# arkworks-rs/poly-commit

Measured on NVIDIA H100. Metric: MarlinKZG10/BLS12-381 commit+open polys/s at deg 2^20, higher is better.
Workload: dtype u32-limb Montgomery (Fq 381-bit x12, Fr 255-bit x8)

## Files before the change

poly-commit_b200/csrc/msm.cuh:

```cuda
#pragma once
#include "ec.cuh"
#include "rt.cuh"

namespace pcgpu {

struct alignas(16) u32x4 { uint32_t x, y, z, w; };

struct MsmGeom {
  uint32_t n;
  uint32_t c;
  uint32_t W;
  uint32_t S;
  uint32_t G;
  uint32_t NB;
  uint32_t TB;
  uint32_t L;
  uint32_t seg_len;
  uint32_t nseg;
  uint32_t scalar_bits;
  uint32_t scalars_mont;
  uint64_t table_stride;
  uint64_t base_off;
  uint32_t affine_rounds;
  uint32_t h_split;
  uint32_t pt_words;
  uint32_t y_words;
  uint32_t pair_tdiv;
};

enum : uint32_t { ENTRY_SIGN = 0x80000000u, ENTRY_GROUP_SHIFT = 26, ENTRY_IDX_MASK = (1u << 26) - 1 };

template <class C>
PCGPU_DEV void load_scalar_plain(const uint32_t *scalars, size_t i, bool mont, uint32_t *k) {
  using R = typename C::Fr;
  const u32x4 *p = reinterpret_cast<const u32x4 *>(scalars) + 2 * i;
  u32x4 lo = p[0], hi = p[1];
  Fp<R> v;
  v.l[0] = lo.x; v.l[1] = lo.y; v.l[2] = lo.z; v.l[3] = lo.w;
  v.l[4] = hi.x; v.l[5] = hi.y; v.l[6] = hi.z; v.l[7] = hi.w;
  if (mont) v = fp_from_mont<R>(v);
#pragma unroll
  for (int j = 0; j < 8; j++) k[j] = v.l[j];
}

template <class C>
PCGPU_DEV bool load_scalar(const uint32_t *scalars, size_t i, bool mont, uint32_t *k, bool *flip) {
  using R = typename C::Fr;
  static_assert(R::N == 8, "256-bit scalar fields only");
  const u32x4 *p = reinterpret_cast<const u32x4 *>(scalars) + 2 * i;
  u32x4 lo = p[0], hi = p[1];
  Fp<R> v;
  v.l[0] = lo.x; v.l[1] = lo.y; v.l[2] = lo.z; v.l[3] = lo.w;
  v.l[4] = hi.x; v.l[5] = hi.y; v.l[6] = hi.z; v.l[7] = hi.w;
  if (mont) v = fp_from_mont<R>(v);
  bool lt_r = false, gt_half = false, decided_r = false, decided_h = false;
#pragma unroll
  for (int j = 7; j >= 0; j--) {
    const uint32_t m = R::mod(j), h = (R::mod(j) >> 1) | (j + 1 < 8 ? R::mod(j + 1 < 8 ? j + 1 : 7) << 31 : 0u);
    if (!decided_r && v.l[j] != m) { lt_r = v.l[j] < m; decided_r = true; }
    if (!decided_h && v.l[j] != h) { gt_half = v.l[j] > h; decided_h = true; }
  }
  *flip = gt_half;
  if (gt_half) {
    Fp<R> m;
#pragma unroll
    for (int j = 0; j < 8; j++) m.l[j] = R::mod(j);
    uint32_t borrow = 0;
#pragma unroll
    for (int j = 0; j < 8; j++) {
      const uint64_t dd = (uint64_t)m.l[j] - v.l[j] - borrow;
      v.l[j] = (uint32_t)dd; borrow = (uint32_t)(dd >> 63);
    }
  }
#pragma unroll
  for (int j = 0; j < 8; j++) k[j] = v.l[j];
  return lt_r;
}

PCGPU_DEV uint32_t scalar_bits_at(const uint32_t *k, uint32_t pos, uint32_t c) {
  uint32_t q = pos >> 5, sh = pos & 31;
  uint64_t lo = q < 8 ? k[q] : 0u;
  uint64_t hi = q + 1 < 8 ? k[q + 1] : 0u;
  uint64_t v = (lo | (hi << 32)) >> sh;
  return (uint32_t)v & ((1u << c) - 1);
}

template <class Fn>
PCGPU_DEV void for_each_digit(const uint32_t *k, const MsmGeom &g, Fn f) {
  uint32_t carry = 0;
  const uint32_t half = 1u << (g.c - 1);
  for (uint32_t w = 0; w < g.W; w++) {
    uint32_t d = scalar_bits_at(k, w * g.c, g.c) + carry;
    bool neg = d > half;
    carry = neg ? 1u : 0u;
    uint32_t mag = neg ? (1u << g.c) - d : d;
    if (mag) f(w, mag, neg);
  }
}

PCGPU_DEV bool scalar_in_range(const uint32_t *k, uint32_t bits) {
  if (bits >= 256) return true;
  uint32_t q = bits >> 5, sh = bits & 31;
  uint32_t o = k[q] >> sh;
  for (uint32_t j = q + 1; j < 8; j++) o |= k[j];
  return o == 0;
}

template <class C>
struct MsmCountBody {
  const uint32_t *scalars; MsmGeom g; uint32_t *counts; uint32_t *err;
  PCGPU_KERNEL_DEV void operator()(size_t i) const {
    uint32_t k[8];
    bool flip;
    if (!load_scalar<C>(scalars, i, g.scalars_mont != 0, k, &flip)) { rt::atomic_or(err, 1u); return; }
    uint32_t *cnt = counts; const MsmGeom gg = g;
    for_each_digit(k, gg, [&](uint32_t w, uint32_t mag, bool) {
      uint32_t s = w % gg.S;
      rt::atomic_add(cnt + (size_t)s * gg.NB + (mag - 1), 1u);
    });
  }
};

template <class C>
struct MsmScatterBody {
  const uint32_t *scalars; MsmGeom g; uint32_t *cursor; uint32_t *entries;
  PCGPU_KERNEL_DEV void operator()(size_t i) const {
    uint32_t k[8];
    bool flip;
    if (!load_scalar<C>(scalars, i, g.scalars_mont != 0, k, &flip)) return;
    uint32_t *cur = cursor; uint32_t *ent = entries; const MsmGeom gg = g;
    for_each_digit(k, gg, [&](uint32_t w, uint32_t mag, bool neg) {
      uint32_t s = w % gg.S, grp = w / gg.S;
      uint32_t pos = rt::atomic_add(cur + (size_t)s * gg.NB + (mag - 1), 1u);
      ent[pos] = ((neg != flip) ? ENTRY_SIGN : 0u) | (grp << ENTRY_GROUP_SHIFT) | (uint32_t)i;
    });
  }
};

enum { SCAN_CHUNK = 256 };
struct ScanChunkSumBody {
  const uint32_t *in; size_t n; uint32_t *partial;
  PCGPU_KERNEL_DEV void operator()(size_t t) const {
    size_t lo = t * SCAN_CHUNK, hi = lo + SCAN_CHUNK < n ? lo + SCAN_CHUNK : n;
    uint32_t s = 0;
    for (size_t i = lo; i < hi; i++) s += in[i];
    partial[t] = s;
  }
};
struct ScanPartialsBody {
  uint32_t *partial; size_t m;
  PCGPU_KERNEL_DEV void operator()(size_t) const {
    uint32_t run = 0;
    for (size_t i = 0; i < m; i++) { uint32_t v = partial[i]; partial[i] = run; run += v; }
    partial[m] = run;
  }
};
struct ScanApplyBody {
  const uint32_t *in; size_t n; const uint32_t *partial; uint32_t *out; size_t m;
  PCGPU_KERNEL_DEV void operator()(size_t t) const {
    size_t lo = t * SCAN_CHUNK, hi = lo + SCAN_CHUNK < n ? lo + SCAN_CHUNK : n;
    uint32_t run = partial[t];
    for (size_t i = lo; i < hi; i++) { uint32_t v = in[i]; out[i] = run; run += v; }
    if (t + 1 == m) out[n] = partial[m];
  }
};

enum { SCAN_BLOCK = 1024, SCAN_PER = 8, SCAN_BLOCK_MAX = 1 << 17 };
struct ScanBlockBody {
  const uint32_t *in; size_t n; uint32_t *out;
  PCGPU_KERNEL_DEV void operator()(size_t, uint32_t *smem) const {
    uint32_t *a = smem, *b = smem + SCAN_BLOCK, *carry = smem + 2 * SCAN_BLOCK;
    PCGPU_BLOCK_FOR(t, 1) { carry[0] = 0; }
    PCGPU_BLOCK_SYNC();
    const size_t tile = (size_t)SCAN_BLOCK * SCAN_PER;
    for (size_t base = 0; base < n; base += tile) {
      PCGPU_BLOCK_FOR(t, SCAN_BLOCK) {
        const size_t lo = base + (size_t)t * SCAN_PER;
        uint32_t sum = 0;
        for (uint32_t k = 0; k < SCAN_PER; k++) if (lo + k < n) sum += in[lo + k];
        a[t] = sum;
      }
      PCGPU_BLOCK_SYNC();
      uint32_t *x = a, *y = b;
      for (uint32_t d = 1; d < SCAN_BLOCK; d <<= 1) {
        PCGPU_BLOCK_FOR(t, SCAN_BLOCK) { y[t] = x[t] + (t >= d ? x[t - d] : 0u); }
        PCGPU_BLOCK_SYNC();
        uint32_t *tmp = x; x = y; y = tmp;
      }
      PCGPU_BLOCK_FOR(t, SCAN_BLOCK) {
        const size_t lo = base + (size_t)t * SCAN_PER;
        uint32_t run = carry[0] + (t ? x[t - 1] : 0u);
        for (uint32_t k = 0; k < SCAN_PER; k++) if (lo + k < n) { uint32_t v = in[lo + k]; out[lo + k] = run; run += v; }
      }
      PCGPU_BLOCK_SYNC();
      PCGPU_BLOCK_FOR(t, 1) { carry[0] += x[SCAN_BLOCK - 1]; }
      PCGPU_BLOCK_SYNC();
    }
    PCGPU_BLOCK_FOR(t, 1) { out[n] = carry[0]; }
  }
};

inline size_t scan_scratch_words(size_t n) { return (n + SCAN_CHUNK - 1) / SCAN_CHUNK + 2; }
inline int exclusive_scan_u32(const uint32_t *in, size_t n, uint32_t *out, uint32_t *scratch, rt::stream_t st) {
  size_t m = (n + SCAN_CHUNK - 1) / SCAN_CHUNK;
  if (m == 0) { return rt::dev_memset(out, 0, sizeof(uint32_t), st); }
  if (n <= SCAN_BLOCK_MAX) return rt::launch_blocks<SCAN_BLOCK>(ScanBlockBody{in, n, out}, 1, (2 * SCAN_BLOCK + 4) * sizeof(uint32_t), st);
  int rc;
  if ((rc = rt::launch<128>(ScanChunkSumBody{in, n, scratch}, m, st))) return rc;
  if ((rc = rt::launch<32>(ScanPartialsBody{scratch, m}, 1, st))) return rc;
  return rt::launch<128>(ScanApplyBody{in, n, scratch, out, m}, m, st);
}

struct TaskCountBody {
  const uint32_t *offsets; uint32_t L; uint32_t *ntasks; uint32_t heavy_min; uint32_t *heavy_count; uint32_t *heavy_list;
  PCGPU_KERNEL_DEV void operator()(size_t b) const {
    uint32_t cnt = offsets[b + 1] - offsets[b];
    uint32_t nt = (cnt + L - 1) / L;
    ntasks[b] = nt;
    if (nt > heavy_min) heavy_list[rt::atomic_add(heavy_count, 1u)] = (uint32_t)b;
  }
};
struct TaskFillBody {
  const uint32_t *task_off; uint32_t *task_bucket;
  PCGPU_KERNEL_DEV void operator()(size_t b) const {
    uint32_t lo = task_off[b], hi = task_off[b + 1];
    for (uint32_t t = lo; t < hi; t++) task_bucket[t] = (uint32_t)b;
  }
};

template <class C>
PCGPU_DEV Affine<C> load_affine(const Affine<C> *p) {
  constexpr int N = coord_words<typename C::F>();
  const u32x4 *q = reinterpret_cast<const u32x4 *>(p);
  Affine<C> a;
  uint32_t tmp[2 * N];
#pragma unroll
  for (int j = 0; j < 2 * N / 4; j++) { u32x4 v = q[j]; tmp[4 * j] = v.x; tmp[4 * j + 1] = v.y; tmp[4 * j + 2] = v.z; tmp[4 * j + 3] = v.w; }
#pragma unroll
  for (int j = 0; j < N; j++) {
    if constexpr (C::EXT == 1) { a.x.l[j] = tmp[j]; a.y.l[j] = tmp[N + j]; }
    else { coord_word(a.x, j) = tmp[j]; coord_word(a.y, j) = tmp[N + j]; }
  }
  return a;
}

template <class C>
PCGPU_DEV const uint32_t *table_record(const uint32_t *tables, size_t idx, const MsmGeom &g) { return tables + idx * g.pt_words; }
template <class C>
PCGPU_DEV Affine<C> load_table_point(const uint32_t *tables, size_t idx, const MsmGeom &g) {
  constexpr int N = coord_words<typename C::F>();
  const uint32_t *rec = tables + idx * g.pt_words;
  const u32x4 *qx = reinterpret_cast<const u32x4 *>(rec), *qy = reinterpret_cast<const u32x4 *>(rec + g.y_words);
  Affine<C> a;
#pragma unroll
  for (int j = 0; j < N / 4; j++) {
    u32x4 v = qx[j]; coord_word(a.x, 4 * j) = v.x; coord_word(a.x, 4 * j + 1) = v.y; coord_word(a.x, 4 * j + 2) = v.z; coord_word(a.x, 4 * j + 3) = v.w;
    u32x4 w = qy[j]; coord_word(a.y, 4 * j) = w.x; coord_word(a.y, 4 * j + 1) = w.y; coord_word(a.y, 4 * j + 2) = w.z; coord_word(a.y, 4 * j + 3) = w.w;
  }
  return a;
}
template <class C>
PCGPU_DEV void store_table_point(uint32_t *tables, size_t idx, uint32_t pt_words, uint32_t y_words, const Affine<C> &a) {
  constexpr int N = coord_words<typename C::F>();
  uint32_t *rec = tables + idx * pt_words;
  u32x4 *qx = reinterpret_cast<u32x4 *>(rec), *qy = reinterpret_cast<u32x4 *>(rec + y_words);
#pragma unroll
  for (int j = 0; j < N / 4; j++) {
    u32x4 v; v.x = coord_word(a.x, 4 * j); v.y = coord_word(a.x, 4 * j + 1); v.z = coord_word(a.x, 4 * j + 2); v.w = coord_word(a.x, 4 * j + 3); qx[j] = v;
    u32x4 w; w.x = coord_word(a.y, 4 * j); w.y = coord_word(a.y, 4 * j + 1); w.z = coord_word(a.y, 4 * j + 2); w.w = coord_word(a.y, 4 * j + 3); qy[j] = w;
  }
}
template <class C> constexpr uint32_t aligned_pt_words() { return C::Fq::N == 12 ? 32u : 2u * C::Fq::N; }
template <class C> constexpr uint32_t aligned_y_words() { return C::Fq::N == 12 ? 16u : (uint32_t)C::Fq::N; }

template <class C>
PCGPU_DEV void store_xyzz(XYZZ<C> *dst, const XYZZ<C> &p) {
  constexpr int N = coord_words<typename C::F>();
  u32x4 *q = reinterpret_cast<u32x4 *>(dst);
  const uint32_t *src = reinterpret_cast<const uint32_t *>(&p);
#pragma unroll
  for (int j = 0; j < 4 * N / 4; j++) { u32x4 v; v.x = src[4 * j]; v.y = src[4 * j + 1]; v.z = src[4 * j + 2]; v.w = src[4 * j + 3]; q[j] = v; }
}

template <class C>
PCGPU_DEV XYZZ<C> load_xyzz(const XYZZ<C> *src) {
  constexpr int N = coord_words<typename C::F>();
  const u32x4 *q = reinterpret_cast<const u32x4 *>(src);
  XYZZ<C> p;
  uint32_t *dst = reinterpret_cast<uint32_t *>(&p);
#pragma unroll
  for (int j = 0; j < 4 * N / 4; j++) { u32x4 v = q[j]; dst[4 * j] = v.x; dst[4 * j + 1] = v.y; dst[4 * j + 2] = v.z; dst[4 * j + 3] = v.w; }
  return p;
}

template <class C>
struct MsmAccumulateBody {
  const uint32_t *tables; MsmGeom g;
  const uint32_t *offsets;
  const uint32_t *task_off;
  const uint32_t *task_bucket;
  const uint32_t *entries;
  XYZZ<C> *partial;
  uint32_t *queue;
  const Affine<C> *pts;
  PCGPU_KERNEL_DEV void operator()(size_t) const {
    const uint32_t total = task_off[g.TB];
    for (;;) {
      uint32_t t = rt::next_task(queue);
      if (t - (t & 31u) >= total) break;
      if (t >= total) continue;
      uint32_t b = task_bucket[t];
      uint32_t t0 = task_off[b], T = task_off[b + 1] - t0, j = t - t0;
      uint32_t base = offsets[b], cnt = offsets[b + 1] - base;
      uint32_t lo = base + (uint32_t)(((uint64_t)cnt * j) / T);
      uint32_t hi = base + (uint32_t)(((uint64_t)cnt * (j + 1)) / T);
      XYZZ<C> acc = XYZZ<C>::inf();
      if (pts) {
        for (uint32_t e = lo; e < hi; e++) { Affine<C> a = load_affine<C>(pts + e); xyzz_madd<C>(acc, a, false); }
      } else {
        for (uint32_t e = lo; e < hi; e++) {
          uint32_t v = entries[e];
          uint32_t grp = (v & ~ENTRY_SIGN) >> ENTRY_GROUP_SHIFT;
          size_t idx = (size_t)grp * g.table_stride + g.base_off + (v & ENTRY_IDX_MASK);
          Affine<C> a = load_table_point<C>(tables, idx, g);
          xyzz_madd<C>(acc, a, (v & ENTRY_SIGN) != 0);
        }
      }
      store_xyzz<C>(partial + t, acc);
    }
  }
};

enum { HEAVY_BUCKET_TASKS = 8, HEAVY_BLOCK = 128, HEAVY_GRID = 64, REDUCE_BLOCK = 128 };

template <class C>
#ifdef __CUDACC__
__device__ __noinline__
#else
inline
#endif
void xyzz_add_ool(XYZZ<C> &acc, const XYZZ<C> &p) { xyzz_add<C>(acc, p); }

template <class C>
struct MsmHeavyBucketBody {
  const uint32_t *task_off; const XYZZ<C> *partial; XYZZ<C> *buckets; const uint32_t *heavy_count; const uint32_t *heavy_list;
  PCGPU_KERNEL_DEV void operator()(size_t blk, uint32_t *smem) const {
    XYZZ<C> *sh = reinterpret_cast<XYZZ<C> *>(smem);
    const uint32_t nheavy = *heavy_count;
    for (uint32_t hb = (uint32_t)blk; hb < nheavy; hb += HEAVY_GRID) {
      const uint32_t b = heavy_list[hb], t0 = task_off[b], t1 = task_off[b + 1];
      PCGPU_BLOCK_FOR(i, HEAVY_BLOCK) {
        XYZZ<C> acc = XYZZ<C>::inf();
#pragma unroll 1
        for (uint32_t q = t0 + i; q < t1; q += HEAVY_BLOCK) { XYZZ<C> p = load_xyzz<C>(partial + q); xyzz_add_ool<C>(acc, p); }
        sh[i] = acc;
      }
      PCGPU_BLOCK_SYNC();
#pragma unroll 1
      for (uint32_t half = HEAVY_BLOCK / 2; half >= 1; half >>= 1) {
        PCGPU_BLOCK_FOR(i, half) { XYZZ<C> x = sh[i], y = sh[i + half]; xyzz_add_ool<C>(x, y); sh[i] = x; }
        PCGPU_BLOCK_SYNC();
      }
      PCGPU_BLOCK_FOR(i, 1) { store_xyzz<C>(buckets + b, sh[0]); }
      PCGPU_BLOCK_SYNC();
    }
  }
};

template <class C>
PCGPU_KERNEL_DEV void block_tree_sum(XYZZ<C> *sh) {
#pragma unroll 1
  for (uint32_t half = REDUCE_BLOCK / 2; half >= 1; half >>= 1) {
    PCGPU_BLOCK_FOR(i, half) { XYZZ<C> x = sh[i], y = sh[i + half]; xyzz_add_ool<C>(x, y); sh[i] = x; }
    PCGPU_BLOCK_SYNC();
  }
}

template <class C>
struct MsmRowReduceBody {
  const uint32_t *task_off; const XYZZ<C> *partial; XYZZ<C> *buckets; XYZZ<C> *Rv;
  uint32_t NB, rows, cols;
  PCGPU_KERNEL_DEV void operator()(size_t blk, uint32_t *smem) const {
    XYZZ<C> *sh = reinterpret_cast<XYZZ<C> *>(smem);
    const uint32_t s = (uint32_t)(blk / rows), hi = (uint32_t)(blk % rows);
    PCGPU_BLOCK_FOR(t, REDUCE_BLOCK) {
      XYZZ<C> acc = XYZZ<C>::inf();
#pragma unroll 1
      for (uint32_t lo = t; lo < cols; lo += REDUCE_BLOCK) {
        const size_t b = (size_t)s * NB + (size_t)hi * cols + lo;
        const uint32_t t0 = task_off[b], t1 = task_off[b + 1];
        XYZZ<C> bs;
        if (t1 - t0 > HEAVY_BUCKET_TASKS) bs = load_xyzz<C>(buckets + b);
        else {
          bs = XYZZ<C>::inf();
#pragma unroll 1
          for (uint32_t q = t0; q < t1; q++) { XYZZ<C> p = load_xyzz<C>(partial + q); xyzz_add_ool<C>(bs, p); }
          store_xyzz<C>(buckets + b, bs);
        }
        xyzz_add_ool<C>(acc, bs);
      }
      sh[t] = acc;
    }
    PCGPU_BLOCK_SYNC();
    block_tree_sum<C>(sh);
    PCGPU_BLOCK_FOR(i, 1) { store_xyzz<C>(Rv + blk, sh[0]); }
  }
};
template <class C>
struct MsmColReduceBody {
  const XYZZ<C> *buckets; XYZZ<C> *Cv;
  uint32_t NB, rows, cols;
  PCGPU_KERNEL_DEV void operator()(size_t blk, uint32_t *smem) const {
    XYZZ<C> *sh = reinterpret_cast<XYZZ<C> *>(smem);
    const uint32_t s = (uint32_t)(blk / cols), lo = (uint32_t)(blk % cols);
    PCGPU_BLOCK_FOR(t, REDUCE_BLOCK) {
      XYZZ<C> acc = XYZZ<C>::inf();
#pragma unroll 1
      for (uint32_t hi = t; hi < rows; hi += REDUCE_BLOCK) {
        XYZZ<C> p = load_xyzz<C>(buckets + (size_t)s * NB + (size_t)hi * cols + lo);
        xyzz_add_ool<C>(acc, p);
      }
      sh[t] = acc;
    }
    PCGPU_BLOCK_SYNC();
    block_tree_sum<C>(sh);
    PCGPU_BLOCK_FOR(i, 1) { store_xyzz<C>(Cv + blk, sh[0]); }
  }
};
template <class C>
struct MsmPlaneReduceBody {
  const XYZZ<C> *Rv, *Cv; XYZZ<C> *plane_out;
  uint32_t rows, cols, bits_c, bits_r;
  PCGPU_KERNEL_DEV void operator()(size_t blk, uint32_t *smem) const {
    XYZZ<C> *sh = reinterpret_cast<XYZZ<C> *>(smem);
    const uint32_t per = bits_c + bits_r;
    const uint32_t s = (uint32_t)(blk / per), j = (uint32_t)(blk % per);
    const bool col = j < bits_c;
    const XYZZ<C> *vals = col ? Cv + (size_t)s * cols : Rv + (size_t)s * rows;
    const uint32_t cnt = col ? cols : rows, wofs = col ? 1u : 0u, bit = col ? j : j - bits_c;
    PCGPU_BLOCK_FOR(t, REDUCE_BLOCK) {
      XYZZ<C> acc = XYZZ<C>::inf();
#pragma unroll 1
      for (uint32_t k = t; k < cnt; k += REDUCE_BLOCK)
        if (((k + wofs) >> bit) & 1) { XYZZ<C> p = load_xyzz<C>(vals + k); xyzz_add_ool<C>(acc, p); }
      sh[t] = acc;
    }
    PCGPU_BLOCK_SYNC();
    block_tree_sum<C>(sh);
    PCGPU_BLOCK_FOR(i, 1) { store_xyzz<C>(plane_out + blk, sh[0]); }
  }
};

}
#include "msm_affine.cuh"
namespace pcgpu {

inline uint32_t ilog2_floor(uint64_t v) { uint32_t l = 0; while (v >>= 1) l++; return l; }

inline uint32_t msm_pick_c(size_t n) {
  uint32_t lg = ilog2_floor(n ? n : 1);
  int c = (int)lg - 4;
  if (c < 8) c = 8;
  if (c > 16) c = 16;
  return (uint32_t)c;
}

inline MsmGeom msm_geometry(size_t n, uint32_t c, uint32_t groups, uint32_t scalar_bits, bool mont,
                            uint64_t table_stride, uint64_t base_off) {
  MsmGeom g;
  g.n = (uint32_t)n; g.c = c;
  g.W = (scalar_bits + c - 1) / c;
  g.G = groups < 1 ? 1 : groups;
  g.S = (g.W + g.G - 1) / g.G;
  g.NB = 1u << (c - 1);
  g.TB = g.S * g.NB;
  g.L = 32;
  if (const char *e = getenv("PCGPU_MSM_L")) { int v = atoi(e); if (v >= 4 && v <= 4096) g.L = (uint32_t)v; }
  g.seg_len = 16;
  g.nseg = (g.NB + g.seg_len - 1) / g.seg_len;
  g.scalar_bits = scalar_bits; g.scalars_mont = mont ? 1 : 0;
  g.table_stride = table_stride; g.base_off = base_off;
  g.affine_rounds = 0;
  g.h_split = (c - 1) / 2;
  g.pt_words = 0; g.y_words = 0;
  g.pair_tdiv = 1;
  return g;
}

inline size_t msm_plane_scratch_elems(const MsmGeom &g) {
  size_t cols = (size_t)1 << g.h_split, rows = g.NB >> g.h_split;
  return (size_t)g.S * (rows + cols);
}

enum {
  MSM_ERR_RANGE = 0,
  MSM_ERR_QUEUE = 8,
  MSM_ERR_HEAVY = 12,
  MSM_ERR_WORDS = 16,
};

#ifndef PCGPU_PAIR_MIN_BLOCKS
#define PCGPU_PAIR_MIN_BLOCKS 4
#endif
enum { PAIR_MIN_BLOCKS = PCGPU_PAIR_MIN_BLOCKS };

template <class C>
int msm_pair_round_oneshot(bool round0, const uint32_t *tables, const MsmGeom &g, const uint32_t *entries, const Affine<C> *in,
                           uint32_t *src, const uint32_t *off_out, uint32_t T, uint32_t *prefix, const uint32_t *pow2, Affine<C> *out,
                           rt::stream_t st) {
  if (round0) return rt::launch_occ<128, PAIR_MIN_BLOCKS>(MsmAffinePairBody<C, true>{tables, g, entries, nullptr, src, off_out, T, prefix, pow2, out}, T, st);
  return rt::launch_occ<128, PAIR_MIN_BLOCKS>(MsmAffinePairBody<C, false>{tables, g, entries, in, src, off_out, T, prefix, pow2, out}, T, st);
}
template <class C> int msm_pair_oneshot_threads(size_t *out) { return rt::resident_threads_occ<128, PAIR_MIN_BLOCKS, MsmAffinePairBody<C, true>>(out); }

template <class C>
int msm_accumulate_launch(const uint32_t *tables, const MsmGeom &g, const uint32_t *offsets, const uint32_t *task_off,
                          const uint32_t *task_bucket, const uint32_t *entries, XYZZ<C> *partial, uint32_t *queue, const Affine<C> *pts,
                          rt::stream_t st) {
  return rt::launch_persistent<128>(MsmAccumulateBody<C>{tables, g, offsets, task_off, task_bucket, entries, partial, queue, pts}, st);
}

template <class C>
int msm_reduce_launch(const MsmGeom &g, const uint32_t *task_off, const XYZZ<C> *partial, XYZZ<C> *buckets, XYZZ<C> *planes,
                      XYZZ<C> *plane_out, const uint32_t *heavy_count, const uint32_t *heavy_list, rt::stream_t st) {
  const uint32_t h = g.h_split, cols = 1u << h, rows = g.NB >> h, bits_c = h + 1, bits_r = g.c - 1 - h;
  const size_t smem = REDUCE_BLOCK * sizeof(XYZZ<C>);
  XYZZ<C> *Rv = planes, *Cv = planes + (size_t)g.S * rows;
  int rc;
  if ((rc = rt::launch_blocks<HEAVY_BLOCK>(MsmHeavyBucketBody<C>{task_off, partial, buckets, heavy_count, heavy_list}, HEAVY_GRID,
                                           HEAVY_BLOCK * sizeof(XYZZ<C>), st))) return rc;
  if ((rc = rt::launch_blocks<REDUCE_BLOCK>(MsmRowReduceBody<C>{task_off, partial, buckets, Rv, g.NB, rows, cols}, (size_t)g.S * rows, smem, st))) return rc;
  if ((rc = rt::launch_blocks<REDUCE_BLOCK>(MsmColReduceBody<C>{buckets, Cv, g.NB, rows, cols}, (size_t)g.S * cols, smem, st))) return rc;
  return rt::launch_blocks<REDUCE_BLOCK>(MsmPlaneReduceBody<C>{Rv, Cv, plane_out, rows, cols, bits_c, bits_r}, (size_t)g.S * (bits_c + bits_r), smem, st);
}

template <class C, class Prof>
inline int msm_run(const uint32_t *tables, const MsmGeom &g, const uint32_t *d_scalars, rt::Arena &arena,
                   const XYZZ<C> **d_planes, size_t *plane_stride, uint32_t **d_err_out, rt::stream_t st, Prof &prof,
                   const uint32_t *pow2 = nullptr, uint32_t *pair_threads = nullptr, uint32_t *pair_tdiv = nullptr) {
  using QF = Fp<typename C::Fq>;
  const size_t max_entries = (size_t)g.n * g.W, max_tasks = max_entries / g.L + g.TB + 1;
  const size_t bound0 = max_entries / 2 + g.TB + 1, bound1 = bound0 / 2 + g.TB + 1;
  const bool pair_rounds = C::EXT == 1 && g.affine_rounds && pow2;
  uint32_t *counts, *offsets, *cursor, *ntasks, *task_off, *task_bucket, *entries, *scratch, *err;
  XYZZ<C> *partial, *buckets, *planes, *plane_out;
  uint32_t *offA = nullptr, *offB = nullptr, *cnt = nullptr, *src = nullptr;
  QF *prefix = nullptr; Affine<C> *ptsA = nullptr, *ptsB = nullptr;
  int rc = arena.carve([&](auto &&buf) {
    buf(counts, g.TB + 2); buf(offsets, g.TB + 2); buf(cursor, g.TB + 2); buf(ntasks, g.TB + 2); buf(task_off, g.TB + 2);
    buf(task_bucket, max_tasks); buf(entries, max_entries + 1); buf(scratch, scan_scratch_words(g.TB + 1)); buf(err, MSM_ERR_WORDS);
    buf(partial, max_tasks); buf(buckets, g.TB); buf(planes, msm_plane_scratch_elems(g));
    buf(plane_out, (size_t)g.S * 2 * g.c);
    if (pair_rounds) {
      buf(offA, g.TB + 2); buf(offB, g.TB + 2); buf(cnt, g.TB + 2); buf(src, bound0);
      buf(prefix, 3 * (bound0 + (1u << 20)));
      buf(ptsA, bound0); buf(ptsB, bound1);
    }
  });
  if (rc) return rc;
  *d_err_out = err; *d_planes = plane_out; *plane_stride = 1;

  prof.begin(0, st);
  if ((rc = rt::dev_memset(counts, 0, (g.TB + 2) * sizeof(uint32_t), st))) return rc;
  if ((rc = rt::dev_memset(err, 0, MSM_ERR_WORDS * sizeof(uint32_t), st))) return rc;
  if ((rc = rt::launch<256>(MsmCountBody<C>{d_scalars, g, counts, err + MSM_ERR_RANGE}, g.n, st))) return rc;
  prof.end(0, st);

  prof.begin(1, st);
  if ((rc = exclusive_scan_u32(counts, g.TB, offsets, scratch, st))) return rc;
  if ((rc = rt::copy_d2d(cursor, offsets, (g.TB + 1) * sizeof(uint32_t), st))) return rc;
  prof.end(1, st);

  prof.begin(2, st);
  if ((rc = rt::launch<256>(MsmScatterBody<C>{d_scalars, g, cursor, entries}, g.n, st))) return rc;
  prof.end(2, st);

  const Affine<C> *pts = nullptr;
  if constexpr (C::EXT == 1) if (pair_rounds) {
    size_t Tmax = 0;
    if ((rc = msm_pair_oneshot_threads<C>(&Tmax))) return rc;
    if (Tmax > (1u << 20)) Tmax = 1u << 20;
    uint32_t tdiv = g.pair_tdiv ? g.pair_tdiv : 1;
    if (const char *e = getenv("PCGPU_MSM_AFFINE_TDIV")) { int v = atoi(e); if (v >= 1 && v <= 16) tdiv = (uint32_t)v; }
    if (tdiv > 1) Tmax = (Tmax / tdiv + 127) / 128 * 128;
    if (pair_threads) *pair_threads = (uint32_t)Tmax;
    if (pair_tdiv) *pair_tdiv = tdiv;
    prof.begin(11, st);
    const uint32_t *off_in = offsets;
    size_t bound = max_entries;
    for (uint32_t r = 0; r < g.affine_rounds; r++) {
      uint32_t *off_out = (r & 1) ? offB : offA;
      Affine<C> *out = (r & 1) ? ptsB : ptsA;
      const Affine<C> *in = (r & 1) ? ptsA : ptsB;
      bound = bound / 2 + g.TB + 1;
      if ((rc = rt::launch<256>(PairCountBody{off_in, cnt}, g.TB, st))) return rc;
      if ((rc = exclusive_scan_u32(cnt, g.TB, off_out, scratch, st))) return rc;
      if ((rc = rt::launch<256>(PairPlanBody{off_in, off_out, g.TB, src}, bound, st))) return rc;
      uint32_t T = (uint32_t)Tmax;
      if (r == 0) prof.begin(12, st);
      rc = msm_pair_round_oneshot<C>(r == 0, tables, g, entries, in, src, off_out, T, (uint32_t *)prefix, pow2, out, st);
      if (rc) return rc;
      if (r == 0) prof.end(12, st);
      off_in = off_out;
      pts = out;
    }
    prof.end(11, st);
    offsets = const_cast<uint32_t *>(off_in);
  }

  prof.begin(3, st);
  if ((rc = rt::dev_memset(err + MSM_ERR_HEAVY, 0, 4, st))) return rc;
  if ((rc = rt::launch<256>(TaskCountBody{offsets, g.L, ntasks, HEAVY_BUCKET_TASKS, err + MSM_ERR_HEAVY, cursor}, g.TB, st))) return rc;
  if ((rc = exclusive_scan_u32(ntasks, g.TB, task_off, scratch, st))) return rc;
  if ((rc = rt::launch<256>(TaskFillBody{task_off, task_bucket}, g.TB, st))) return rc;
  prof.end(3, st);

  prof.begin(4, st);
  if ((rc = msm_accumulate_launch<C>(tables, g, offsets, task_off, task_bucket, entries, partial, err + MSM_ERR_QUEUE, pts, st))) return rc;
  prof.end(4, st);

  prof.begin(5, st);
  if ((rc = msm_reduce_launch<C>(g, task_off, partial, buckets, planes, plane_out, err + MSM_ERR_HEAVY, cursor, st))) return rc;
  prof.end(5, st);
  return rt::OK;
}

}
```

poly-commit_b200/csrc/msm_affine.cuh:

```cuda
#pragma once
#include "msm.cuh"

namespace pcgpu {

enum : uint32_t { PAIR_SINGLE = 0x80000000u, PAIR_EXC = 0x40000000u, PAIR_NONE = 0xffffffffu };

struct PairCountBody {
  const uint32_t *off_in; uint32_t *cnt_out;
  PCGPU_KERNEL_DEV void operator()(size_t b) const { cnt_out[b] = (off_in[b + 1] - off_in[b] + 1) / 2; }
};

struct PairPlanBody {
  const uint32_t *off_in; const uint32_t *off_out; uint32_t TB; uint32_t *src;
  PCGPU_KERNEL_DEV void operator()(size_t o) const {
    if (o >= off_out[TB]) return;
    uint32_t lo = 0, hi = TB;
    while (hi - lo > 1) { uint32_t mid = (lo + hi) / 2; if (off_out[mid] <= (uint32_t)o) lo = mid; else hi = mid; }
    uint32_t b = lo, j = (uint32_t)o - off_out[b], cnt = off_in[b + 1] - off_in[b];
    uint32_t first = off_in[b] + 2 * j;
    src[o] = first | ((2 * j + 1 >= cnt) ? PAIR_SINGLE : 0u);
  }
};

PCGPU_DEV u32x4 ldg4(const u32x4 *p) {
#ifdef __CUDA_ARCH__
  uint4 v = __ldg(reinterpret_cast<const uint4 *>(p));
  u32x4 r; r.x = v.x; r.y = v.y; r.z = v.z; r.w = v.w; return r;
#else
  return *p;
#endif
}
PCGPU_DEV uint32_t ldg_plain(const uint32_t *p) { return *p; }
PCGPU_DEV uint32_t ldg1(const uint32_t *p) {
#ifdef __CUDA_ARCH__
  return __ldg(p);
#else
  return *p;
#endif
}
template <class Q>
PCGPU_DEV Fp<Q> load_fq(const uint32_t *p) {
  constexpr int N = Q::N;
  const u32x4 *q = reinterpret_cast<const u32x4 *>(p);
  Fp<Q> r;
#pragma unroll
  for (int j = 0; j < N / 4; j++) { u32x4 v = ldg4(q + j); r.l[4 * j] = v.x; r.l[4 * j + 1] = v.y; r.l[4 * j + 2] = v.z; r.l[4 * j + 3] = v.w; }
  return r;
}
template <class Q>
PCGPU_DEV void store_fq(uint32_t *p, const Fp<Q> &a) {
  constexpr int N = Q::N;
  u32x4 *q = reinterpret_cast<u32x4 *>(p);
#pragma unroll
  for (int j = 0; j < N / 4; j++) { u32x4 v; v.x = a.l[4 * j]; v.y = a.l[4 * j + 1]; v.z = a.l[4 * j + 2]; v.w = a.l[4 * j + 3]; q[j] = v; }
}

enum : uint32_t { PK_ADD = 0, PK_DBL = 1, PK_TAKE_P = 2, PK_TAKE_Q = 3, PK_INF = 4 };
template <class C>
PCGPU_DEV uint32_t pair_classify(const Affine<C> &P, const Affine<C> &Qp, bool single, Fp<typename C::Fq> &d) {
  using Q = typename C::Fq;
  d = Fp<Q>::one();
  if (single) return PK_TAKE_P;
  if (P.is_inf()) return Qp.is_inf() ? PK_INF : PK_TAKE_Q;
  if (Qp.is_inf()) return PK_TAKE_P;
  if (P.x == Qp.x) {
    if (P.y == Qp.y && !P.y.is_zero()) { d = fp_dbl<Q>(P.y); return PK_DBL; }
    return PK_INF;
  }
  d = fp_sub<Q>(Qp.x, P.x);
  return PK_ADD;
}

template <class C, bool FROM_TABLES>
struct MsmAffinePairBody {
  const uint32_t *tables; MsmGeom g; const uint32_t *entries;
  const Affine<C> *pts_in;
  uint32_t *src; const uint32_t *off_out;
  uint32_t T;
  uint32_t *prefix;
  const uint32_t *pow2;
  Affine<C> *pts_out;

  struct Slot { uint32_t a, b; };
  PCGPU_DEV Slot fetch_slot(uint32_t o) const {
    uint32_t sv = ldg1(src + o);
    uint32_t i0 = sv & ~(PAIR_SINGLE | PAIR_EXC);
    bool single = (sv & PAIR_SINGLE) != 0;
    Slot s;
    if (FROM_TABLES) { s.a = ldg1(entries + i0); s.b = single ? PAIR_NONE : ldg1(entries + i0 + 1); }
    else { s.a = i0; s.b = single ? PAIR_NONE : 0u; }
    return s;
  }
  PCGPU_DEV const uint32_t *slot_rec(uint32_t v) const {
    uint32_t grp = (v & ~ENTRY_SIGN) >> ENTRY_GROUP_SHIFT;
    return table_record<C>(tables, (size_t)grp * g.table_stride + g.base_off + (v & ENTRY_IDX_MASK), g);
  }
  PCGPU_DEV Fp<typename C::Fq> slot_x(const Slot &s, int which) const {
    using Q = typename C::Fq;
    if (FROM_TABLES) return load_fq<Q>(slot_rec(which ? s.b : s.a));
    return load_fq<Q>(reinterpret_cast<const uint32_t *>(pts_in + s.a + which));
  }
  PCGPU_DEV Affine<C> slot_point(const Slot &s, int which) const {
    using Q = typename C::Fq;
    if (FROM_TABLES) {
      uint32_t v = which ? s.b : s.a;
      const uint32_t *rec = slot_rec(v);
      Affine<C> a; a.x = load_fq<Q>(rec); a.y = load_fq<Q>(rec + g.y_words);
      if (!a.is_inf()) a.y = fp_cneg<Q>(a.y, (v & ENTRY_SIGN) != 0);
      return a;
    }
    return load_affine<C>(pts_in + s.a + which);
  }
  PCGPU_DEV Fp<typename C::Fq> slot_denominator(const Slot &s) const {
    using Q = typename C::Fq;
    if (s.b == PAIR_NONE) return Fp<Q>::one();
    Fp<Q> x1 = slot_x(s, 0), x2 = slot_x(s, 1);
    if (x1 != x2 && !x1.is_zero() && !x2.is_zero()) return fp_sub<Q>(x2, x1);
    Affine<C> P = slot_point(s, 0), Qp = slot_point(s, 1);
    Fp<Q> d;
    pair_classify<C>(P, Qp, false, d);
    return d;
  }

  PCGPU_KERNEL_DEV void operator()(size_t t) const {
    using Q = typename C::Fq;
    constexpr int N = Q::N;
    if (t >= T) return;
    const uint32_t total = off_out[g.TB];
    uint32_t *xbuf = prefix + (size_t)T * N * ((total + T - 1) / T);
    uint32_t *dbuf = xbuf + (size_t)T * N * ((total + T - 1) / T);
    const uint32_t kmax = (uint32_t)t < total ? (total - (uint32_t)t + T - 1) / T : 0u;
    Fp<Q> acc = Fp<Q>::one();
    {
      Slot nxt; nxt.a = 0; nxt.b = PAIR_NONE;
      if (kmax) nxt = fetch_slot((uint32_t)t);
      for (uint32_t k = 0; k < kmax; k++) {
        Slot cur = nxt;
        if (k + 1 < kmax) nxt = fetch_slot((k + 1) * T + (uint32_t)t);
        Fp<Q> d;
        if (FROM_TABLES) {
          Fp<Q> x1 = slot_x(cur, 0);
          bool exc = false;
          if (cur.b == PAIR_NONE) d = Fp<Q>::one();
          else {
            Fp<Q> x2 = slot_x(cur, 1);
            if (x1 != x2 && !x1.is_zero() && !x2.is_zero()) d = fp_sub<Q>(x2, x1);
            else { Affine<C> P = slot_point(cur, 0), Qp = slot_point(cur, 1); pair_classify<C>(P, Qp, false, d); exc = true; }
          }
          if (exc) src[k * T + (uint32_t)t] |= PAIR_EXC;
          store_fq<Q>(xbuf + ((size_t)k * T + t) * N, x1);
          store_fq<Q>(dbuf + ((size_t)k * T + t) * N, d);
        } else {
          d = slot_denominator(cur);
        }
        store_fq<Q>(prefix + ((size_t)k * T + t) * N, acc);
        acc = fp_mul<Q>(acc, d);
      }
    }
    Fp<Q> inv = fp_inv_gcd<Q>(acc, pow2);
    Slot nxt2; nxt2.a = 0; nxt2.b = PAIR_NONE;
    if (kmax) nxt2 = fetch_slot((kmax - 1) * T + (uint32_t)t);
    for (uint32_t k2 = kmax; k2-- > 0;) {
      const uint32_t k = k2;
      uint32_t o = k * T + (uint32_t)t;
      Slot cur = nxt2;
      const bool exc = FROM_TABLES && (ldg_plain(src + o) & PAIR_EXC) != 0;
      if (k > 0) nxt2 = fetch_slot(o - T);
      bool single = cur.b == PAIR_NONE;
      if (FROM_TABLES && !exc) {
        Fp<Q> x1 = load_fq<Q>(xbuf + ((size_t)k * T + t) * N), d = load_fq<Q>(dbuf + ((size_t)k * T + t) * N);
        Fp<Q> y1 = fp_cneg<Q>(load_fq<Q>(slot_rec(cur.a) + g.y_words), (cur.a & ENTRY_SIGN) != 0);
        Fp<Q> dinv = fp_mul<Q>(inv, load_fq<Q>(prefix + ((size_t)k * T + t) * N));
        inv = fp_mul<Q>(inv, d);
        Affine<C> R;
        if (single) { R.x = x1; R.y = y1; if (x1.is_zero() && y1.is_zero()) R = Affine<C>::inf(); }
        else {
          Fp<Q> y2 = fp_cneg<Q>(load_fq<Q>(slot_rec(cur.b) + g.y_words), (cur.b & ENTRY_SIGN) != 0);
          Fp<Q> lam = fp_mul<Q>(fp_sub<Q>(y2, y1), dinv);
          Fp<Q> x2 = fp_add<Q>(x1, d);
          Fp<Q> x3 = fp_sub<Q>(fp_sub<Q>(fp_sqr<Q>(lam), x1), x2);
          R.x = x3;
          R.y = fp_sub<Q>(fp_mul<Q>(lam, fp_sub<Q>(x1, x3)), y1);
        }
        Affine<C> *dst0 = pts_out + o;
        store_fq<Q>(reinterpret_cast<uint32_t *>(dst0), R.x);
        store_fq<Q>(reinterpret_cast<uint32_t *>(dst0) + N, R.y);
        continue;
      }
      Affine<C> P = slot_point(cur, 0), Qp = single ? Affine<C>::inf() : slot_point(cur, 1);
      Fp<Q> d;
      uint32_t kind = pair_classify<C>(P, Qp, single, d);
      Fp<Q> dinv = fp_mul<Q>(inv, load_fq<Q>(prefix + ((size_t)k * T + t) * N));
      inv = fp_mul<Q>(inv, d);
      Affine<C> R;
      if (kind == PK_ADD || kind == PK_DBL) {
        Fp<Q> num = kind == PK_ADD ? fp_sub<Q>(Qp.y, P.y) : fp_mul3<Q>(fp_sqr<Q>(P.x));
        Fp<Q> lam = fp_mul<Q>(num, dinv);
        Fp<Q> x3 = fp_sub<Q>(fp_sub<Q>(fp_sqr<Q>(lam), P.x), kind == PK_ADD ? Qp.x : P.x);
        R.x = x3;
        R.y = fp_sub<Q>(fp_mul<Q>(lam, fp_sub<Q>(P.x, x3)), P.y);
      } else if (kind == PK_TAKE_P) R = P;
      else if (kind == PK_TAKE_Q) R = Qp;
      else R = Affine<C>::inf();
      Affine<C> *dst = pts_out + o;
      store_fq<Q>(reinterpret_cast<uint32_t *>(dst), R.x);
      store_fq<Q>(reinterpret_cast<uint32_t *>(dst) + N, R.y);
    }
  }
};

}
```

poly-commit_b200/csrc/rt.cuh:

```cuda
#pragma once
#include <stddef.h>
#include <stdint.h>
#include <stdlib.h>
#include <string.h>
#include <atomic>
#include <type_traits>

#ifndef PCGPU_EMUL
#include <cuda_runtime.h>
#endif

namespace pcgpu {
namespace rt {

enum : int {
  OK = 0,
  E_CUDA = -1,
  E_OOM = -2,
  E_BADARG = -3,
  E_LEN = -4,
  E_RANGE = -5,
  E_DEGREE = -6,
  E_HIDING = -7,
};

inline std::atomic<uint64_t> &launch_counter() { static std::atomic<uint64_t> c{0}; return c; }

#ifdef PCGPU_EMUL
typedef void *stream_t;
inline int dev_malloc(void **p, size_t bytes) { *p = ::malloc(bytes ? bytes : 1); return *p ? OK : E_OOM; }
inline void dev_free(void *p) { ::free(p); }
inline int dev_memset(void *p, int v, size_t bytes, stream_t) { memset(p, v, bytes); return OK; }
inline int copy_h2d(void *d, const void *h, size_t bytes, stream_t) { memcpy(d, h, bytes); return OK; }
inline int copy_d2h(void *h, const void *d, size_t bytes, stream_t) { memcpy(h, d, bytes); return OK; }
inline int copy_d2d(void *d, const void *s, size_t bytes, stream_t) { memmove(d, s, bytes); return OK; }
inline int copy_d2h_2d(void *h, size_t hpitch, const void *d, size_t dpitch, size_t width, size_t rows, stream_t) {
  for (size_t r = 0; r < rows; r++) memcpy((char *)h + r * hpitch, (const char *)d + r * dpitch, width);
  return OK;
}
inline int stream_sync(stream_t) { return OK; }
inline int last_error() { return OK; }
typedef int event_t;
inline int event_create(event_t *e) { *e = 0; return OK; }
inline void event_destroy(event_t) {}
inline int event_record(event_t, stream_t) { return OK; }
inline int stream_wait_event(stream_t, event_t) { return OK; }
inline int host_alloc_pinned(void **p, size_t bytes) { *p = ::malloc(bytes ? bytes : 1); return *p ? OK : E_OOM; }
inline void host_free_pinned(void *p) { ::free(p); }

template <int BLOCK, class Body>
inline int launch(const Body &body, size_t n, stream_t) {
  for (size_t i = 0; i < n; i++) body(i);
  return OK;
}
template <class T> inline T atomic_add(T *p, T v) { T o = *p; *p = o + v; return o; }
template <class T> inline T atomic_or(T *p, T v) { T o = *p; *p = o | v; return o; }
#define PCGPU_KERNEL_DEV inline
inline uint32_t next_task(uint32_t *counter) { return atomic_add(counter, 1u); }
template <int BLOCK, class Body>
inline int launch_persistent(const Body &body, stream_t) { body(0); return OK; }
template <int BLOCK, class Body> inline int resident_threads(size_t *out) { *out = 48; return OK; }
template <int BLOCK, int MINB, class Body> inline int launch_occ(const Body &body, size_t n, stream_t s) { return launch<BLOCK>(body, n, s); }
template <int BLOCK, int MINB, class Body> inline int resident_threads_occ(size_t *out) { *out = 48; return OK; }
#define PCGPU_BLOCK_FOR(i, n) for (uint32_t i = 0; i < (uint32_t)(n); i++)
#define PCGPU_BLOCK_SYNC() do { } while (0)
#define PCGPU_WARP_ANY(x) (x)
template <int BLOCK, class Body>
inline int launch_blocks(const Body &body, size_t nblocks, size_t smem_bytes, stream_t) {
  uint32_t *smem = (uint32_t *)::malloc(smem_bytes ? smem_bytes : 16);
  if (!smem) return E_OOM;
  for (size_t b = 0; b < nblocks; b++) body(b, smem);
  ::free(smem);
  return OK;
}

template <int BLOCK, int MINB, class Body>
inline int launch_blocks_occ(const Body &body, size_t nblocks, size_t smem_bytes, stream_t s) { return launch_blocks<BLOCK>(body, nblocks, smem_bytes, s); }

#else
typedef cudaStream_t stream_t;

inline int map_cuda(cudaError_t e) {
  if (e == cudaSuccess) return OK;
  if (e == cudaErrorMemoryAllocation) return E_OOM;
  return E_CUDA;
}
inline int dev_malloc(void **p, size_t bytes) { return map_cuda(cudaMalloc(p, bytes ? bytes : 1)); }
inline void dev_free(void *p) { if (p) cudaFree(p); }
inline int dev_memset(void *p, int v, size_t bytes, stream_t s) { return map_cuda(cudaMemsetAsync(p, v, bytes, s)); }
inline int copy_h2d(void *d, const void *h, size_t bytes, stream_t s) { return map_cuda(cudaMemcpyAsync(d, h, bytes, cudaMemcpyHostToDevice, s)); }
inline int copy_d2h(void *h, const void *d, size_t bytes, stream_t s) { return map_cuda(cudaMemcpyAsync(h, d, bytes, cudaMemcpyDeviceToHost, s)); }
inline int copy_d2d(void *d, const void *s_, size_t bytes, stream_t s) { return map_cuda(cudaMemcpyAsync(d, s_, bytes, cudaMemcpyDeviceToDevice, s)); }
inline int copy_d2h_2d(void *h, size_t hpitch, const void *d, size_t dpitch, size_t width, size_t rows, stream_t s) {
  return map_cuda(cudaMemcpy2DAsync(h, hpitch, d, dpitch, width, rows, cudaMemcpyDeviceToHost, s));
}
inline int stream_sync(stream_t s) { return map_cuda(cudaStreamSynchronize(s)); }
inline int last_error() { return map_cuda(cudaGetLastError()); }
typedef cudaEvent_t event_t;
inline int event_create(event_t *e) { return map_cuda(cudaEventCreateWithFlags(e, cudaEventDisableTiming)); }
inline void event_destroy(event_t e) { cudaEventDestroy(e); }
inline int event_record(event_t e, stream_t s) { return map_cuda(cudaEventRecord(e, s)); }
inline int stream_wait_event(stream_t s, event_t e) { return map_cuda(cudaStreamWaitEvent(s, e, 0)); }
inline int host_alloc_pinned(void **p, size_t bytes) { return map_cuda(cudaMallocHost(p, bytes ? bytes : 1)); }
inline void host_free_pinned(void *p) { if (p) cudaFreeHost(p); }

template <class Body, int BLOCK>
__global__ void __launch_bounds__(BLOCK) run_kernel(const Body body, size_t n) {
  size_t tid = (size_t)blockIdx.x * BLOCK + threadIdx.x;
  if (tid < n) body(tid);
}

template <int BLOCK, class Body>
inline int launch(const Body &body, size_t n, stream_t s) {
  if (n == 0) return OK;
  size_t grid = (n + BLOCK - 1) / BLOCK;
  run_kernel<Body, BLOCK><<<(unsigned)grid, BLOCK, 0, s>>>(body, n);
  launch_counter().fetch_add(1, std::memory_order_relaxed);
  return last_error();
}
template <class Body, int BLOCK, int MINB>
__global__ void __launch_bounds__(BLOCK, MINB) run_kernel_occ(const Body body, size_t n) {
  size_t tid = (size_t)blockIdx.x * BLOCK + threadIdx.x;
  if (tid < n) body(tid);
}
template <int BLOCK, int MINB, class Body>
inline int launch_occ(const Body &body, size_t n, stream_t s) {
  if (n == 0) return OK;
  size_t grid = (n + BLOCK - 1) / BLOCK;
  run_kernel_occ<Body, BLOCK, MINB><<<(unsigned)grid, BLOCK, 0, s>>>(body, n);
  launch_counter().fetch_add(1, std::memory_order_relaxed);
  return last_error();
}
template <int BLOCK, int MINB, class Body>
inline int resident_threads_occ(size_t *out) {
  static size_t cached = 0;
  if (!cached) {
    int dev = 0, sms = 0, per_sm = 0;
    cudaError_t e = cudaGetDevice(&dev);
    if (e == cudaSuccess) e = cudaDeviceGetAttribute(&sms, cudaDevAttrMultiProcessorCount, dev);
    if (e == cudaSuccess) e = cudaOccupancyMaxActiveBlocksPerMultiprocessor(&per_sm, run_kernel_occ<Body, BLOCK, MINB>, BLOCK, 0);
    if (e != cudaSuccess) return map_cuda(e);
    cached = (size_t)sms * (per_sm > 0 ? per_sm : 1) * BLOCK;
  }
  *out = cached;
  return OK;
}
#define PCGPU_BLOCK_FOR(i, n) for (uint32_t i = threadIdx.x; i < (uint32_t)(n); i += blockDim.x)
#define PCGPU_BLOCK_SYNC() __syncthreads()
#define PCGPU_WARP_ANY(x) __any_sync(0xffffffffu, (x))
template <class Body, int BLOCK>
__global__ void __launch_bounds__(BLOCK) run_block_kernel(const Body body) {
  extern __shared__ uint4 pcgpu_smem[];
  body((size_t)blockIdx.x, reinterpret_cast<uint32_t *>(pcgpu_smem));
}
template <int BLOCK, class Body>
inline int launch_blocks(const Body &body, size_t nblocks, size_t smem_bytes, stream_t s) {
  if (nblocks == 0) return OK;
  if (smem_bytes > 48 * 1024) {
    cudaError_t e = cudaFuncSetAttribute(run_block_kernel<Body, BLOCK>, cudaFuncAttributeMaxDynamicSharedMemorySize, (int)smem_bytes);
    if (e != cudaSuccess) return map_cuda(e);
  }
  run_block_kernel<Body, BLOCK><<<(unsigned)nblocks, BLOCK, smem_bytes, s>>>(body);
  launch_counter().fetch_add(1, std::memory_order_relaxed);
  return last_error();
}
template <class Body, int BLOCK, int MINB>
__global__ void __launch_bounds__(BLOCK, MINB) run_block_kernel_occ(const Body body) {
  extern __shared__ uint4 pcgpu_smem[];
  body((size_t)blockIdx.x, reinterpret_cast<uint32_t *>(pcgpu_smem));
}
template <int BLOCK, int MINB, class Body>
inline int launch_blocks_occ(const Body &body, size_t nblocks, size_t smem_bytes, stream_t s) {
  if (nblocks == 0) return OK;
  if (smem_bytes > 48 * 1024) {
    cudaError_t e = cudaFuncSetAttribute(run_block_kernel_occ<Body, BLOCK, MINB>, cudaFuncAttributeMaxDynamicSharedMemorySize, (int)smem_bytes);
    if (e != cudaSuccess) return map_cuda(e);
  }
  run_block_kernel_occ<Body, BLOCK, MINB><<<(unsigned)nblocks, BLOCK, smem_bytes, s>>>(body);
  launch_counter().fetch_add(1, std::memory_order_relaxed);
  return last_error();
}
__device__ __forceinline__ uint32_t next_task(uint32_t *counter) {
  uint32_t lane = threadIdx.x & 31, base = 0;
  if (lane == 0) base = atomicAdd(counter, 32u);
  base = __shfl_sync(0xffffffffu, base, 0);
  return base + lane;
}
template <class Body, int BLOCK>
__global__ void __launch_bounds__(BLOCK) run_persistent_kernel(const Body body) {
  body((size_t)blockIdx.x * BLOCK + threadIdx.x);
}
template <int BLOCK, class Body>
inline int resident_threads(size_t *out) {
  static size_t cached = 0;
  if (!cached) {
    int dev = 0, sms = 0, per_sm = 0;
    cudaError_t e = cudaGetDevice(&dev);
    if (e == cudaSuccess) e = cudaDeviceGetAttribute(&sms, cudaDevAttrMultiProcessorCount, dev);
    if (e == cudaSuccess) e = cudaOccupancyMaxActiveBlocksPerMultiprocessor(&per_sm, run_kernel<Body, BLOCK>, BLOCK, 0);
    if (e != cudaSuccess) return map_cuda(e);
    cached = (size_t)sms * (per_sm > 0 ? per_sm : 1) * BLOCK;
  }
  *out = cached;
  return OK;
}
template <int BLOCK, class Body>
inline int launch_persistent(const Body &body, stream_t s) {
  static int grid = 0;
  if (grid == 0) {
    int dev = 0, sms = 0, per_sm = 0;
    cudaError_t e = cudaGetDevice(&dev);
    if (e == cudaSuccess) e = cudaDeviceGetAttribute(&sms, cudaDevAttrMultiProcessorCount, dev);
    if (e == cudaSuccess) e = cudaOccupancyMaxActiveBlocksPerMultiprocessor(&per_sm, run_persistent_kernel<Body, BLOCK>, BLOCK, 0);
    if (e != cudaSuccess) return map_cuda(e);
    grid = sms * (per_sm > 0 ? per_sm : 1);
  }
  run_persistent_kernel<Body, BLOCK><<<grid, BLOCK, 0, s>>>(body);
  launch_counter().fetch_add(1, std::memory_order_relaxed);
  return last_error();
}
template <class T> __device__ __forceinline__ T atomic_add(T *p, T v) { return atomicAdd(p, v); }
template <class T> __device__ __forceinline__ T atomic_or(T *p, T v) { return atomicOr(p, v); }
#define PCGPU_KERNEL_DEV __device__ __forceinline__
#endif

struct Arena {
  char *base = nullptr;
  size_t cap = 0;
  int reserve(size_t bytes) {
    if (bytes <= cap) return OK;
    if (base) dev_free(base);
    base = nullptr; cap = 0;
    int rc = dev_malloc((void **)&base, bytes);
    if (rc) return rc;
    cap = bytes;
    return OK;
  }
  template <class List> int carve(const List &list) {
    size_t used = 0;
    list([&](auto *&p, size_t count) { used += padded(sizeof *p, count); });
    int rc = reserve(used);
    if (rc) return rc;
    used = 0;
    list([&](auto *&p, size_t count) {
      p = reinterpret_cast<std::remove_reference_t<decltype(p)>>(base + used);
      used += padded(sizeof *p, count);
    });
    return OK;
  }
  static size_t padded(size_t elem, size_t count) { size_t b = elem * count; return ((b ? b : 1) + 255) & ~(size_t)255; }
  void release() { if (base) dev_free(base); base = nullptr; cap = 0; }
};

}
}
```

Baseline: 72.28.

## Share one field inversion per block via shared-memory product tree in affine pair kernel

Each thread in the affine pair-add batch kernel used to run its own GCD field inversion on its accumulated product. The kernel now builds a product tree of the per-thread accumulators in shared memory, inverts only the root once per block, and walks back down the tree to give each thread its own inverse. This trades 128 inversions per block for about 3×128 Montgomery multiplications, log-depth block syncs and about 12 KB of shared memory. The extra shared memory and the serial single-thread inversion could lower occupancy or leave the rest of the block idle while it runs.

```diff
diff --git a/poly-commit_b200/csrc/msm.cuh b/poly-commit_b200/csrc/msm.cuh
--- a/poly-commit_b200/csrc/msm.cuh
+++ b/poly-commit_b200/csrc/msm.cuh
@@ -508,10 +508,16 @@
 int msm_pair_round_oneshot(bool round0, const uint32_t *tables, const MsmGeom &g, const uint32_t *entries, const Affine<C> *in,
                            uint32_t *src, const uint32_t *off_out, uint32_t T, uint32_t *prefix, const uint32_t *pow2, Affine<C> *out,
                            rt::stream_t st) {
-  if (round0) return rt::launch_occ<128, PAIR_MIN_BLOCKS>(MsmAffinePairBody<C, true>{tables, g, entries, nullptr, src, off_out, T, prefix, pow2, out}, T, st);
-  return rt::launch_occ<128, PAIR_MIN_BLOCKS>(MsmAffinePairBody<C, false>{tables, g, entries, in, src, off_out, T, prefix, pow2, out}, T, st);
-}
-template <class C> int msm_pair_oneshot_threads(size_t *out) { return rt::resident_threads_occ<128, PAIR_MIN_BLOCKS, MsmAffinePairBody<C, true>>(out); }
+  using B0 = MsmAffinePairBody<C, true>;
+  using B1 = MsmAffinePairBody<C, false>;
+  const size_t blocks = (T + PAIR_BLOCK - 1) / PAIR_BLOCK;
+  if (round0) return rt::launch_blocks_occ<PAIR_BLOCK, PAIR_MIN_BLOCKS>(B0{tables, g, entries, nullptr, src, off_out, T, prefix, pow2, out}, blocks, B0::smem_bytes(), st);
+  return rt::launch_blocks_occ<PAIR_BLOCK, PAIR_MIN_BLOCKS>(B1{tables, g, entries, in, src, off_out, T, prefix, pow2, out}, blocks, B1::smem_bytes(), st);
+}
+template <class C> int msm_pair_oneshot_threads(size_t *out) {
+  using B0 = MsmAffinePairBody<C, true>;
+  return rt::resident_block_threads_occ<PAIR_BLOCK, PAIR_MIN_BLOCKS, B0>(B0::smem_bytes(), out);
+}
 
 template <class C>
 int msm_accumulate_launch(const uint32_t *tables, const MsmGeom &g, const uint32_t *offsets, const uint32_t *task_off,
diff --git a/poly-commit_b200/csrc/msm_affine.cuh b/poly-commit_b200/csrc/msm_affine.cuh
--- a/poly-commit_b200/csrc/msm_affine.cuh
+++ b/poly-commit_b200/csrc/msm_affine.cuh
@@ -4,6 +4,7 @@
 namespace pcgpu {
 
 enum : uint32_t { PAIR_SINGLE = 0x80000000u, PAIR_EXC = 0x40000000u, PAIR_NONE = 0xffffffffu };
+enum : uint32_t { PAIR_BLOCK = 128 };
 
 struct PairCountBody {
   const uint32_t *off_in; uint32_t *cnt_out;
@@ -45,6 +46,15 @@
   Fp<Q> r;
 #pragma unroll
   for (int j = 0; j < N / 4; j++) { u32x4 v = ldg4(q + j); r.l[4 * j] = v.x; r.l[4 * j + 1] = v.y; r.l[4 * j + 2] = v.z; r.l[4 * j + 3] = v.w; }
+  return r;
+}
+template <class Q>
+PCGPU_DEV Fp<Q> load_sh(const uint32_t *p) {
+  constexpr int N = Q::N;
+  const u32x4 *q = reinterpret_cast<const u32x4 *>(p);
+  Fp<Q> r;
+#pragma unroll
+  for (int j = 0; j < N / 4; j++) { u32x4 v = q[j]; r.l[4 * j] = v.x; r.l[4 * j + 1] = v.y; r.l[4 * j + 2] = v.z; r.l[4 * j + 3] = v.w; }
   return r;
 }
 template <class Q>
@@ -122,14 +132,40 @@
     return d;
   }
 
-  PCGPU_KERNEL_DEV void operator()(size_t t) const {
+  static constexpr size_t smem_bytes() { return (2 * PAIR_BLOCK - 1) * C::Fq::N * sizeof(uint32_t); }
+  PCGPU_KERNEL_DEV void operator()(size_t blk, uint32_t *tree) const {
     using Q = typename C::Fq;
     constexpr int N = Q::N;
-    if (t >= T) return;
-    const uint32_t total = off_out[g.TB];
+    const uint32_t total = off_out[g.TB], t0 = (uint32_t)blk * PAIR_BLOCK;
+    auto node = [&](uint32_t i) { return tree + (size_t)i * N; };
+    PCGPU_BLOCK_FOR(i, PAIR_BLOCK) { store_fq<Q>(node(PAIR_BLOCK - 1 + i), pass1(t0 + i, total)); }
+    PCGPU_BLOCK_SYNC();
+    for (uint32_t w = PAIR_BLOCK / 2; w >= 1; w >>= 1) {
+      PCGPU_BLOCK_FOR(j, w) { uint32_t p = w - 1 + j; store_fq<Q>(node(p), fp_mul<Q>(load_sh<Q>(node(2 * p + 1)), load_sh<Q>(node(2 * p + 2)))); }
+      PCGPU_BLOCK_SYNC();
+    }
+    PCGPU_BLOCK_FOR(j, 1) { store_fq<Q>(node(0), fp_inv_gcd<Q>(load_sh<Q>(node(0)), pow2)); }
+    PCGPU_BLOCK_SYNC();
+    for (uint32_t w = 1; w <= PAIR_BLOCK / 2; w <<= 1) {
+      PCGPU_BLOCK_FOR(j, w) {
+        uint32_t p = w - 1 + j;
+        Fp<Q> I = load_sh<Q>(node(p)), L = load_sh<Q>(node(2 * p + 1)), R = load_sh<Q>(node(2 * p + 2));
+        store_fq<Q>(node(2 * p + 1), fp_mul<Q>(I, R));
+        store_fq<Q>(node(2 * p + 2), fp_mul<Q>(I, L));
+      }
+      PCGPU_BLOCK_SYNC();
+    }
+    PCGPU_BLOCK_FOR(i, PAIR_BLOCK) { pass2(t0 + i, total, load_sh<Q>(node(PAIR_BLOCK - 1 + i))); }
+  }
+
+  PCGPU_KERNEL_DEV uint32_t slot_count(uint32_t t, uint32_t total) const { return t < T && t < total ? (total - t + T - 1) / T : 0u; }
+
+  PCGPU_KERNEL_DEV Fp<typename C::Fq> pass1(uint32_t t, uint32_t total) const {
+    using Q = typename C::Fq;
+    constexpr int N = Q::N;
     uint32_t *xbuf = prefix + (size_t)T * N * ((total + T - 1) / T);
     uint32_t *dbuf = xbuf + (size_t)T * N * ((total + T - 1) / T);
-    const uint32_t kmax = (uint32_t)t < total ? (total - (uint32_t)t + T - 1) / T : 0u;
+    const uint32_t kmax = slot_count(t, total);
     Fp<Q> acc = Fp<Q>::one();
     {
       Slot nxt; nxt.a = 0; nxt.b = PAIR_NONE;
@@ -157,7 +193,15 @@
         acc = fp_mul<Q>(acc, d);
       }
     }
-    Fp<Q> inv = fp_inv_gcd<Q>(acc, pow2);
+    return acc;
+  }
+
+  PCGPU_KERNEL_DEV void pass2(uint32_t t, uint32_t total, Fp<typename C::Fq> inv) const {
+    using Q = typename C::Fq;
+    constexpr int N = Q::N;
+    uint32_t *xbuf = prefix + (size_t)T * N * ((total + T - 1) / T);
+    uint32_t *dbuf = xbuf + (size_t)T * N * ((total + T - 1) / T);
+    const uint32_t kmax = slot_count(t, total);
     Slot nxt2; nxt2.a = 0; nxt2.b = PAIR_NONE;
     if (kmax) nxt2 = fetch_slot((kmax - 1) * T + (uint32_t)t);
     for (uint32_t k2 = kmax; k2-- > 0;) {
diff --git a/poly-commit_b200/csrc/rt.cuh b/poly-commit_b200/csrc/rt.cuh
--- a/poly-commit_b200/csrc/rt.cuh
+++ b/poly-commit_b200/csrc/rt.cuh
@@ -62,6 +62,7 @@
 template <int BLOCK, class Body> inline int resident_threads(size_t *out) { *out = 48; return OK; }
 template <int BLOCK, int MINB, class Body> inline int launch_occ(const Body &body, size_t n, stream_t s) { return launch<BLOCK>(body, n, s); }
 template <int BLOCK, int MINB, class Body> inline int resident_threads_occ(size_t *out) { *out = 48; return OK; }
+template <int BLOCK, int MINB, class Body> inline int resident_block_threads_occ(size_t, size_t *out) { *out = 48; return OK; }
 #define PCGPU_BLOCK_FOR(i, n) for (uint32_t i = 0; i < (uint32_t)(n); i++)
 #define PCGPU_BLOCK_SYNC() do { } while (0)
 #define PCGPU_WARP_ANY(x) (x)
@@ -179,6 +180,20 @@
   run_block_kernel_occ<Body, BLOCK, MINB><<<(unsigned)nblocks, BLOCK, smem_bytes, s>>>(body);
   launch_counter().fetch_add(1, std::memory_order_relaxed);
   return last_error();
+}
+template <int BLOCK, int MINB, class Body>
+inline int resident_block_threads_occ(size_t smem_bytes, size_t *out) {
+  static size_t cached = 0;
+  if (!cached) {
+    int dev = 0, sms = 0, per_sm = 0;
+    cudaError_t e = cudaGetDevice(&dev);
+    if (e == cudaSuccess) e = cudaDeviceGetAttribute(&sms, cudaDevAttrMultiProcessorCount, dev);
+    if (e == cudaSuccess) e = cudaOccupancyMaxActiveBlocksPerMultiprocessor(&per_sm, run_block_kernel_occ<Body, BLOCK, MINB>, BLOCK, smem_bytes);
+    if (e != cudaSuccess) return map_cuda(e);
+    cached = (size_t)sms * (per_sm > 0 ? per_sm : 1) * BLOCK;
+  }
+  *out = cached;
+  return OK;
 }
 __device__ __forceinline__ uint32_t next_task(uint32_t *counter) {
   uint32_t lane = threadIdx.x & 31, base = 0;
```

Result: no change. 72.40, median of 6 (+0.2%).
